# keith2018/TinyGPT

Hardware: AMD Instinct MI355X
Metric: decode tokens/sec (and % HBM roofline), Llama-3.2-1B bf16 batch=1, 1 GPU (higher is better)
Workload: dtype bf16; 1 GPU; Llama-3.2-1B bf16, batch 1 per GPU: 2048-token prefill then greedy decode (one step = one token, context 2054..3411); replicas=1, params=1235814400, graph=True

## Files before the change

### include/tgx.h

```cpp
#ifndef TGX_H
#define TGX_H

#include <stdint.h>

#ifdef __cplusplus
extern "C" {
#endif

#define TGX_ABI_VERSION 3

#if defined(__GNUC__)
#define TGX_API __attribute__((visibility("default")))
#else
#define TGX_API
#endif

typedef struct tgx_ctx tgx_ctx;

typedef enum tgx_status {
  TGX_OK = 0,
  TGX_ERR_INVALID = 1,
  TGX_ERR_UNSUPPORTED = 2,
  TGX_ERR_DEVICE = 3,
  TGX_ERR_STATE = 4,
// ... 132 lines not shown
#define TGX_KERNEL_LMHEAD 5
#define TGX_KERNEL_COUNT 6
TGX_API int tgx_profile_decode(tgx_ctx* ctx, int n_reps, int64_t* launches ,
                       double* total_ms );

TGX_API int tgx_read_probs(tgx_ctx* ctx, float* out);

TGX_API int tgx_set_logits(tgx_ctx* ctx, const float* logits, int batch);

TGX_API int tgx_set_option(tgx_ctx* ctx, const char* key, int value);

TGX_API int tgx_get_option(const tgx_ctx* ctx, const char* key, int* out_value);

TGX_API int64_t tgx_bytes_per_token(const tgx_ctx* ctx, int64_t T);

TGX_API int tgx_abi_version(void);

#ifdef __cplusplus
}
#endif
#endif
```

### tinygpt_amd/csrc/abi.hip

```cpp
#include <climits>
#include "ctx.h"
#include "kernels/kv_fork.h"
#include "kernels/kv_pack.h"
#include "row_snapshot.h"

static std::string g_create_err;

int set_err(tgx_ctx* c, int code, const char* fmt, ...) {
  char buf[512];
  va_list ap;
  va_start(ap, fmt);
  vsnprintf(buf, sizeof buf, fmt, ap);
  va_end(ap);
  if (c) c->err = buf; else g_create_err = buf;
  return code;
}

namespace {

inline uint16_t host_f32_to_bf16(float f) {
  uint32_t u;
  memcpy(&u, &f, 4);
  if ((u & 0x7fffffffu) > 0x7f800000u) return (uint16_t)((u >> 16) | 0x40);
  u += 0x7fffu + ((u >> 16) & 1u);
// ... 2093 lines not shown
  }
  return set_err(c, TGX_ERR_INVALID, "unknown option %s", key);
}

int64_t tgx_bytes_per_token(const tgx_ctx* c, int64_t T) {
  if (!c) return -1;
  const tgx_model_desc& d = c->d;
  const int64_t H = d.hidden, I = d.inter, V = d.vocab, L = d.layers, q = (int64_t)d.heads * d.head_dim, kv = (int64_t)d.kv_heads * d.head_dim;
  const int64_t b = (int64_t)c->esz;
  if (c->gpt2) {
    const int64_t per_layer = 3 * H * H + 3 * H + H * H + H + I * H + I + H * I + H + 4 * H;
    return b * (L * per_layer + 2 * H + H + V * H) + b * 2 * L * kv * T;
  }
  const int64_t per_layer = (q + 2 * kv) * H + (d.qkv_bias ? (q + 2 * kv) : 0) + H * q + 2 * I * H + H * I + 2 * H;
  int64_t saved = 0;
  auto packed_saving = [&](const PackedMat& m, int64_t rows, int64_t cols) { if (m.P) saved += b * rows * cols - rows * (m.row_bytes + 16); };
  for (const LayerW& w : c->L) { packed_saving(w.pgu, 2 * I, H); packed_saving(w.pdown, H, I); }
  packed_saving(c->plm, V, H);
  return b * (L * per_layer + H + V * H) + b * 2 * L * kv * T - saved;
}

}
```

### tinygpt_amd/csrc/ctx.h

```cpp
#pragma once
#include <hip/hip_runtime.h>

#include <algorithm>
#include <cmath>
#include <cstdarg>
#include <cstdio>
#include <cstdlib>
#include <cstring>
#include <string>
#include <vector>

#include "../../include/tgx.h"
#include "kernels/common.h"
#include "kv_pool.h"
#include "dev_mem.h"

using tgx::bf16_t;
typedef unsigned char ebyte;

namespace tgx { struct SampScratch; struct LpRecord; struct LpRow; }

constexpr int MAX_TICKET_EVENTS = 64;
constexpr int HOST_RING = 256;

struct PackedMat {
  unsigned char* P = nullptr;
  tgx::u32x4* rec = nullptr;
  long long row_bytes = 0;
  unsigned int base2 = 0;
  int ks = 0;
  int max_row_esc = 0;
  long long n_esc = 0;
};

struct LayerW {
  ebyte *in_norm = nullptr, *post_norm = nullptr;
  ebyte *wqkv = nullptr, *bqkv = nullptr, *wo = nullptr, *wgu = nullptr, *wdown = nullptr;
  PackedMat pgu, pdown;
  ebyte *q_norm = nullptr, *k_norm = nullptr;
  bool q_norm_ok = false, k_norm_ok = false;
  int merged_filled = 0;
  bool in_norm_ok = false, post_norm_ok = false, wo_ok = false, wdown_ok = false;
  ebyte *in_norm_b = nullptr, *post_norm_b = nullptr, *bo = nullptr, *bfc = nullptr, *bdown = nullptr;
  int gpt2_filled = 0;
// ... 260 lines not shown
template <typename T>
int dev_grow(tgx_ctx* c, T** p, size_t* bytes, size_t need) {
  if (need <= *bytes) return TGX_OK;
  HIP_OK(c, hipStreamSynchronize(c->stream));
  void* q = *p; const bool ok = c->mem.grow(&q, bytes, need); *p = static_cast<T*>(q);
  return ok ? TGX_OK : set_err(c, TGX_ERR_DEVICE, "dev_grow to %zu bytes failed: %s", need, hipGetErrorString(hipPeekAtLastError()));
}

namespace tgx { struct AttnArgs; struct FinalizeArgs; struct AttnPrefillArgs; struct RopeKvArgs; }

void drop_step_graphs(tgx_ctx* c);
int kv_ensure_blocks(tgx_ctx* c, int row, long long tokens);
bool is_greedy(const tgx_sampler_cfg* s);
bool row_records(const tgx_ctx* c, int row);
int gemv_grid(const tgx_ctx* c, int units, int ks, int bpc);
int pack_weights(tgx_ctx* c);
bool oproj_sliced_ok(const tgx_ctx* c, int R, long long kv_stride);
bool oproj_fused_capable(const tgx_ctx* c);
bool oproj_fused_ok(const tgx_ctx* c, int R, long long kv_stride);
int launch_layer_kernel(tgx_ctx* c, RowState* rv, int R, int l, int cls, float* resid, long long kv_stride);
void launch_layers(tgx_ctx* c, RowState* rv, int R, long long kv_stride);
void launch_layers(tgx_ctx* c, int row0, int R);
void launch_lm_head(tgx_ctx* c, int row0, int R);
void launch_lm_head_at(tgx_ctx* c, const float* x, float* logits, float* part_val, int* part_idx, int R);
tgx::FinalizeArgs make_finalize_args(tgx_ctx* c, int row, bool advance_pos, bool log_step);
void launch_finalize_greedy(tgx_ctx* c, int row0, int R, bool advance_pos, bool log_step);
void launch_finalize_rows(tgx_ctx* c, int row0, int M);
void launch_embed_chunk(tgx_ctx* c, const long long* ids, int R, int pos0);
void launch_add_pos(tgx_ctx* c, int* pos, int n);
void launch_argmax_partials(tgx_ctx* c, const float* logits, int V, float* part_val, int* part_idx);
// ... 47 lines not shown
```

### tinygpt_amd/csrc/decode.hip

```cpp
#include "ctx.h"
#include "kernels/attn_decode.h"
#include "kernels/gemv.h"
#include "kernels/gemv_packed.h"
#include "kernels/oproj_sliced.h"
#include "kernels/verify.h"

int gemv_grid(const tgx_ctx* c, int units, int ks, int bpc) {
  const int upb = 4 / ks;
  const int want = (units + upb - 1) / upb;
  const int cap = c->num_cus * bpc;
  return want < cap ? want : cap;
}

static int gemv_nx(int K, int ks) { return ((K / 8) + ks * 64 - 1) / (ks * 64); }

static int gemv_auto_ks(int K, int want) {
  int ks = want;
  while (ks < 4 && gemv_nx(K, ks) > 8) ks *= 2;
  return ks;
}

static tgx::GemvArgs gemv_row(const tgx_ctx* c, tgx::GemvArgs a, int r) {
  a.x += (size_t)r * a.x_stride;
  if (a.out) a.out += (size_t)r * a.out_stride;
// ... 20 lines not shown
  for (int r = 0; r < R; r++) hipLaunchKernelGGL((tgx::gemv_kernel<DT, PRO, EPI, NX, 1>), g, b, 0, c->stream, gemv_row(c, a, r));
}

template <int PRO, int EPI, int NX>
static void launch_gemv_packed_nx(tgx_ctx* c, const tgx::GemvPackedArgs& p, int grid) {
  const dim3 g(grid), b(256);
  if constexpr (EPI != tgx::EPI_LOGITS) {
    if (p.g.x_acc || p.g.res_acc) { hipLaunchKernelGGL((tgx::gemv_packed_kernel<PRO, EPI, NX, true>), g, b, p.g.x_acc ? (size_t)p.g.K * 4 : 0, c->stream, p); return; }
  }
  hipLaunchKernelGGL((tgx::gemv_packed_kernel<PRO, EPI, NX, false>), g, b, 0, c->stream, p);
}

template <int PRO, int EPI>
static void launch_gemv_packed(tgx_ctx* c, const tgx::GemvArgs& a, const PackedMat& pk, int grid, int nx) {
  tgx::GemvPackedArgs p{};
  p.g = a; p.P = pk.P; p.rec = pk.rec; p.row_bytes = pk.row_bytes; p.base2 = pk.base2;
  switch (nx) {
    case 1: launch_gemv_packed_nx<PRO, EPI, 1>(c, p, grid); break;
    case 2: launch_gemv_packed_nx<PRO, EPI, 2>(c, p, grid); break;
    case 3: launch_gemv_packed_nx<PRO, EPI, 3>(c, p, grid); break;
    case 4: launch_gemv_packed_nx<PRO, EPI, 4>(c, p, grid); break;
    case 5: launch_gemv_packed_nx<PRO, EPI, 5>(c, p, grid); break;
    case 6: launch_gemv_packed_nx<PRO, EPI, 6>(c, p, grid); break;
    case 7: launch_gemv_packed_nx<PRO, EPI, 7>(c, p, grid); break;
    default: launch_gemv_packed_nx<PRO, EPI, 8>(c, p, grid); break;
  }
}

static int pack_matrix(tgx_ctx* c, const ebyte* W, int N, int K, int cls, int* stat_dev, PackedMat* out) {
  const int ks = gemv_auto_ks(K, c->tune[cls].ks), nx = gemv_nx(K, ks);
  if (K % 8 || K > tgx::PACKED_K_MAX || nx > 8) return TGX_OK;
  PackedMat m;
  m.ks = ks; m.row_bytes = (long long)ks * ((nx + 3) / 4) * 3072;
  int rc;
  if ((rc = dev_alloc(c, &m.P, (size_t)N * (size_t)m.row_bytes)) || (rc = dev_alloc(c, &m.rec, (size_t)N))) { dev_free(c, &m.P); return rc; }
  HIP_OK(c, hipMemsetAsync(stat_dev, 0, 4 * sizeof(int), c->stream));
  const size_t n8 = (size_t)N * K / 8;
  hipLaunchKernelGGL(tgx::packed_maxexp_kernel, dim3((unsigned)std::min<size_t>((n8 + 255) / 256, 4096)), dim3(256), 0, c->stream, reinterpret_cast<const bf16_t*>(W), n8, stat_dev);
  tgx::PackRowsArgs a{};
  a.W = reinterpret_cast<const bf16_t*>(W); a.N = N; a.K = K; a.ks = ks; a.nx = nx; a.P = m.P; a.rec = m.rec; a.row_bytes = m.row_bytes; a.stat = stat_dev;
  hipLaunchKernelGGL(tgx::pack_rows_kernel, dim3(N), dim3(64), 0, c->stream, a);
  int stat[4] = {0, 0, 0, 0};
  HIP_OK(c, hipGetLastError());
  HIP_OK(c, hipMemcpyAsync(stat, stat_dev, sizeof(stat), hipMemcpyDeviceToHost, c->stream));
  HIP_OK(c, hipStreamSynchronize(c->stream));
  c->packed_max_row_esc = std::max(c->packed_max_row_esc, stat[3]);
  if (stat[1] > 0) {
    dev_free(c, &m.P); dev_free(c, &m.rec);
    c->packed_fallbacks++;
    return TGX_OK;
  }
  const unsigned int E0 = (unsigned int)std::max(stat[0] - 15, 0);
  m.base2 = (E0 << 7) | (E0 << 23); m.n_esc = stat[2]; m.max_row_esc = stat[3];
  *out = m;
  c->packed_matrices++;
  return TGX_OK;
}

int pack_weights(tgx_ctx* c) {
  const tgx_model_desc& d = c->d;
  if (!c->weights_packed || c->dt != tgx::DT_BF16 || c->gpt2) return TGX_OK;
  int* stat_dev = nullptr;
  int rc = dev_alloc(c, &stat_dev, 4);
  for (size_t l = 0; l < c->L.size() && !rc; l++) {
    LayerW& w = c->L[l];
    if (c->packed_classes & 1) rc = pack_matrix(c, w.wgu, 2 * d.inter, d.hidden, TGX_KERNEL_GATEUP, stat_dev, &w.pgu);
    if (!rc && (c->packed_classes & 2) && d.inter <= 16384) rc = pack_matrix(c, w.wdown, d.hidden, d.inter, TGX_KERNEL_DOWN, stat_dev, &w.pdown);
  }
  if (!rc && (c->packed_classes & 4)) rc = pack_matrix(c, d.tied ? c->embed : c->lm_head, d.vocab, d.hidden, TGX_KERNEL_LMHEAD, stat_dev, &c->plm);
  dev_free(c, &stat_dev);
// ... 254 lines not shown
```

### tinygpt_amd/csrc/kernels/gemv_packed.h

```cpp
#pragma once
#include "gemv.h"

namespace tgx {

constexpr int PACKED_ESC = 4;
constexpr int PACKED_K_MAX = 32768;

struct PackedQuad { u32x4 s01, s23, c; };

struct GemvPackedArgs {
  GemvArgs g;
  const unsigned char* P;
  const u32x4* rec;
  long long row_bytes;
  unsigned int base2;
};

__device__ __forceinline__ bool packed_has_escape(unsigned int C) { return ((C - 0x11111111u) & ~C & 0x88888888u) != 0; }

__device__ __forceinline__ Slice8<DT_BF16> packed_decode(unsigned int S0, unsigned int S1, unsigned int C, unsigned int base2, const u32x4 rec, int chunk) {
  Slice8<DT_BF16> o;
  o.v[0] = ((S0 & 0x007f007fu) | ((S0 << 8) & 0x80008000u)) + ((( C        & 0x000f000fu) << 7) + base2);
  o.v[1] = (((S0 >> 8) & 0x007f007fu) | (S0 & 0x80008000u)) + ((((C >> 4)  & 0x000f000fu) << 7) + base2);
  o.v[2] = ((S1 & 0x007f007fu) | ((S1 << 8) & 0x80008000u)) + ((((C >> 8)  & 0x000f000fu) << 7) + base2);
  o.v[3] = (((S1 >> 8) & 0x007f007fu) | (S1 & 0x80008000u)) + ((((C >> 12) & 0x000f000fu) << 7) + base2);
  if (packed_has_escape(C)) {
#pragma unroll
    for (int e = 0; e < PACKED_ESC; e++) {
      const unsigned int en = rec[e];
      const unsigned int t = (en >> 16) & 7u, sh = (t & 1u) << 4;
      const unsigned int dsel = (en >> 19) == (unsigned int)chunk ? (t >> 1) : 4u;
      const unsigned int m = 0xffffu << sh, val = (en & 0xffffu) << sh;
#pragma unroll
      for (int dd = 0; dd < 4; dd++) o.v[dd] = dsel == (unsigned int)dd ? ((o.v[dd] & ~m) | val) : o.v[dd];
    }
  }
  return o;
}

template <int PRO, int EPI, int NX, bool XACC = false>
__global__ __launch_bounds__(256, NX <= 4 ? 4 : 1) void gemv_packed_kernel(const GemvPackedArgs pa) {
  constexpr int DT = DT_BF16;
  constexpr int NQ = (NX + 3) / 4;
  typedef elem_t<DT> E;
  static_assert(PRO == PRO_PLAIN || PRO == PRO_RMSNORM, "packed forms: plain or RMSNorm prologue");
  static_assert(EPI == EPI_SILU_MUL || EPI == EPI_RESIDUAL || EPI == EPI_LOGITS, "packed forms: gate_up, down, lm_head");
  const GemvArgs& a = pa.g;
  const int n_wg = (int)gridDim.x;
  __shared__ float ps[4][2];
  __shared__ float sv[1][4];
  __shared__ int si[1][4];

  const int lane = threadIdx.x & 63, wv = threadIdx.x >> 6;
  const int KS = a.ks, UPB = 4 / KS;
  const int slot = wv / KS, kpart = wv - slot * KS;
  const int nchunk = a.K >> 3;
  const int per = ((nchunk + KS * 64 - 1) / (KS * 64)) * 64;
  const int c_begin = min(kpart * per, nchunk), c_end = min(c_begin + per, nchunk);
  const int stride = n_wg * UPB;

  int cidx[NX];
  bool cok[NX];
#pragma unroll
  for (int j = 0; j < NX; j++) {
    const int c = c_begin + lane + 64 * j;
    cok[j] = c < c_end;
    cidx[j] = cok[j] ? c : max(c_end - 1, 0);
  }

  const size_t lane_off = (size_t)kpart * NQ * 3072 + (size_t)lane * 16;
  PackedQuad wa[NQ], wb[NQ], na[NQ], nb[NQ];
  u32x4 ea, eb, nea = {}, neb = {};
  auto load_unit = [&](int ub, PackedQuad* ta, PackedQuad* tb, u32x4& ra_rec, u32x4& rb_rec) {
    const int u = min(ub + slot, a.units - 1);
    int ra, rb; bool v;
    unit_rows<EPI>(a, u, ra, rb, v);
    ra_rec = pa.rec[ra]; rb_rec = pa.rec[rb];
    const unsigned char* pra = pa.P + (size_t)ra * pa.row_bytes + lane_off;
    const unsigned char* prb = pa.P + (size_t)rb * pa.row_bytes + lane_off;
#pragma unroll
    for (int q = 0; q < NQ; q++) {
      const u32x4* qa = reinterpret_cast<const u32x4*>(pra + (size_t)q * 3072);
      const u32x4* qb = reinterpret_cast<const u32x4*>(prb + (size_t)q * 3072);
      ta[q].s01 = load_nt(qa); ta[q].s23 = load_nt(qa + 64); ta[q].c = load_nt(qa + 128);
      tb[q].s01 = load_nt(qb); tb[q].s23 = load_nt(qb + 64); tb[q].c = load_nt(qb + 128);
    }
  };
  auto rec_uniform = [](const u32x4 v) {
    return u32x4{(unsigned int)__builtin_amdgcn_readfirstlane((int)v[0]), (unsigned int)__builtin_amdgcn_readfirstlane((int)v[1]),
                 (unsigned int)__builtin_amdgcn_readfirstlane((int)v[2]), (unsigned int)__builtin_amdgcn_readfirstlane((int)v[3])};
  };

  float xr[NX][8];
  auto load_x = [&]() {
    const f32x4* xg = reinterpret_cast<const f32x4*>(a.x);
#pragma unroll
    for (int j = 0; j < NX; j++) {
      f32x4 v0 = xg[2 * cidx[j]], v1 = xg[2 * cidx[j] + 1];
      if (!cok[j]) { v0 = f32x4{0.f, 0.f, 0.f, 0.f}; v1 = v0; }
#pragma unroll
      for (int t = 0; t < 4; t++) { xr[j][t] = v0[t]; xr[j][4 + t] = v1[t]; }
    }
  };
  ulonglong2 xacc0[(XACC && PRO == PRO_RMSNORM) ? 4 : 1];
  if constexpr (XACC && PRO == PRO_RMSNORM) {
    const ulonglong2* ag = reinterpret_cast<const ulonglong2*>(a.x_acc + (size_t)min((int)threadIdx.x, nchunk - 1) * 8);
#pragma unroll
    for (int q = 0; q < 4; q++) xacc0[q] = ag[q];
    __builtin_amdgcn_sched_barrier(0);
  }
  int ub = blockIdx.x * UPB;
  if (ub < a.units) load_unit(ub, wa, wb, nea, neb);
  Slice8<DT> nw_x[(XACC && PRO == PRO_RMSNORM) ? NX : 1];
  if constexpr (XACC && PRO == PRO_RMSNORM) {
#pragma unroll
    for (int j = 0; j < NX; j++) nw_x[j] = load_slice<DT>(static_cast<const E*>(a.norm_w), cidx[j]);
    __builtin_amdgcn_sched_barrier(0);
  }

  if constexpr (XACC && PRO == PRO_RMSNORM) {
    extern __shared__ __attribute__((aligned(16))) float xs[];
    for (int cs = threadIdx.x; cs < nchunk; cs += 256) {
      ulonglong2 t[4];
      if (cs == (int)threadIdx.x) {
#pragma unroll
        for (int q = 0; q < 4; q++) t[q] = xacc0[q];
      } else {
// ... 46 lines not shown
      slice_unpack<DT>(nw[j], w);
#pragma unroll
      for (int t = 0; t < 8; t++) xr[j][t] = w[t] * (xr[j][t] * inv);
    }
  }

  if constexpr (PRO != PRO_PLAIN) {
    if (a.act16) {
#pragma unroll
      for (int j = 0; j < NX; j++)
#pragma unroll
        for (int t = 0; t < 8; t++) xr[j][t] = elem_to_f32<DT>(f32_to_elem<DT>(xr[j][t]));
    }
  }

  float best_val = -INFINITY;
  int best_idx = 0x7fffffff;
  ea = rec_uniform(nea); eb = rec_uniform(neb);

  for (; ub < a.units; ub += stride) {
    const bool has_next = ub + stride < a.units;
    if (has_next) load_unit(ub + stride, na, nb, nea, neb);

    const int u = ub + slot;
    const bool writer = u < a.units && kpart == 0 && lane == 0;
    int ra = 0, rb = 0; bool rb_valid = false;
    float e0 = 0.f, e1 = 0.f;
    if (writer) {
      unit_rows<EPI>(a, u, ra, rb, rb_valid);
      if (EPI == EPI_RESIDUAL) {
        if constexpr (XACC) { e0 = fix_to_f32(a.res_acc[ra]); e1 = fix_to_f32(a.res_acc[rb]); }
        else { e0 = a.out[ra]; e1 = a.out[rb]; }
      }
    }

    float acc_a0 = 0.f, acc_b0 = 0.f, acc_a1 = 0.f, acc_b1 = 0.f;
#pragma unroll
    for (int j = 0; j < NX; j++) {
      const f32x4 xa = f32x4{xr[j][0], xr[j][1], xr[j][2], xr[j][3]};
      const f32x4 xb = f32x4{xr[j][4], xr[j][5], xr[j][6], xr[j][7]};
      const int q = j >> 2, jj = j & 3;
      const u32x4 sa4 = (jj & 2) ? wa[q].s23 : wa[q].s01, sb4 = (jj & 2) ? wb[q].s23 : wb[q].s01;
      const int chunk = c_begin + lane + 64 * j;
      const Slice8<DT> da = packed_decode(sa4[(jj & 1) * 2], sa4[(jj & 1) * 2 + 1], wa[q].c[jj], pa.base2, ea, chunk);
      const Slice8<DT> db = packed_decode(sb4[(jj & 1) * 2], sb4[(jj & 1) * 2 + 1], wb[q].c[jj], pa.base2, eb, chunk);
      if (j & 1) { acc_a1 = dot8<DT>(acc_a1, da, xa, xb); acc_b1 = dot8<DT>(acc_b1, db, xa, xb); }
      else       { acc_a0 = dot8<DT>(acc_a0, da, xa, xb); acc_b0 = dot8<DT>(acc_b0, db, xa, xb); }
    }
    float sa = wave_sum(acc_a0 + acc_a1);
    float sb = wave_sum(acc_b0 + acc_b1);

    if (KS > 1) {
      __syncthreads();
      if (lane == 0) { ps[wv][0] = sa; ps[wv][1] = sb; }
      __syncthreads();
      if (kpart == 0) {
        sa = ps[slot * KS][0]; sb = ps[slot * KS][1];
        for (int k = 1; k < KS; k++) { sa += ps[slot * KS + k][0]; sb += ps[slot * KS + k][1]; }
      }
    }

    if (writer) {
      float va = sa, vb = sb;
      if (EPI == EPI_LOGITS) {
        a.logits[ra] = va;
// ... 2 lines not shown
          a.logits[rb] = vb;
          if (vb > best_val) { best_val = vb; best_idx = rb; }
        }
      } else {
        if (a.bias) { const E* bias = static_cast<const E*>(a.bias); va += elem_to_f32<DT>(bias[ra]); vb += elem_to_f32<DT>(bias[rb]); }
        if (EPI == EPI_RESIDUAL) {
          a.out[ra] = e0 + va;
          if (rb_valid) a.out[rb] = e1 + vb;
          if constexpr (XACC) { a.res_acc[ra] = 0; if (rb_valid) a.res_acc[rb] = 0; }
        } else if (EPI == EPI_SILU_MUL) {
          a.out[u] = round_storage_if<DT>((va / (1.0f + expf(-va))) * vb, a.act16);
        }
      }
    }

#pragma unroll
    for (int q = 0; q < NQ; q++) { wa[q] = na[q]; wb[q] = nb[q]; }
    ea = rec_uniform(nea); eb = rec_uniform(neb);
  }

  if (EPI == EPI_LOGITS) {
    if (lane == 0) { sv[0][wv] = best_val; si[0][wv] = best_idx; }
    __syncthreads();
    if (threadIdx.x == 0) {
      float bv = sv[0][0]; int bi = si[0][0];
      for (int w = 1; w < 4; w++)
        if (sv[0][w] > bv || (sv[0][w] == bv && si[0][w] < bi)) { bv = sv[0][w]; bi = si[0][w]; }
      a.part_val[blockIdx.x] = bv;
      a.part_idx[blockIdx.x] = bi;
    }
  }
}

// ... 3 lines not shown
    const u32x4 v = reinterpret_cast<const u32x4*>(W)[i];
#pragma unroll
    for (int t = 0; t < 4; t++) {
      const int e0 = (v[t] >> 7) & 0xff, e1 = (v[t] >> 23) & 0xff;
      if (e0 < 255) m = max(m, e0);
      if (e1 < 255) m = max(m, e1);
    }
  }
#pragma unroll
  for (int o = 32; o > 0; o >>= 1) m = max(m, __shfl_xor(m, o, 64));
  if ((threadIdx.x & 63) == 0) atomicMax(stat, m);
}

struct PackRowsArgs {
  const bf16_t* W;
  int N, K, ks, nx;
  unsigned char* P;
  u32x4* rec;
  long long row_bytes;
  int* stat;
};

__global__ __launch_bounds__(64) void pack_rows_kernel(const PackRowsArgs a) {
  __shared__ unsigned int ent[PACKED_ESC];
  const int row = blockIdx.x, lane = threadIdx.x;
  const int E0 = max(a.stat[0] - 15, 0);
  const bf16_t* w = a.W + (size_t)row * a.K;
  if (lane < PACKED_ESC) ent[lane] = 0xffffffffu;
  __syncthreads();
  int cnt = 0;
  for (int k0 = 0; k0 < a.K; k0 += 64) {
    const int k = k0 + lane;
    unsigned int bits = 0; bool esc = false;
    if (k < a.K) { bits = w[k]; const int code = (int)((bits >> 7) & 0xff) - E0; esc = code < 1 || code > 15; }
    const unsigned long long bal = __ballot(esc);
    const int p = cnt + __popcll(bal & ((1ull << lane) - 1ull));
    if (esc && p < PACKED_ESC) ent[p] = ((unsigned int)k << 16) | bits;
    cnt += __popcll(bal);
  }
  __syncthreads();
  if (lane == 0) {
    a.rec[row] = u32x4{ent[0], ent[1], ent[2], ent[3]};
    if (cnt > PACKED_ESC) atomicAdd(a.stat + 1, 1);
    if (cnt) { atomicAdd(a.stat + 2, cnt); atomicMax(a.stat + 3, cnt); }
  }
  const int nchunk = a.K >> 3, nq = (a.nx + 3) / 4;
  const int per = ((nchunk + a.ks * 64 - 1) / (a.ks * 64)) * 64;
  for (int p = 0; p < a.ks; p++) {
    const int c_begin = min(p * per, nchunk), c_end = min(c_begin + per, nchunk);
    for (int q = 0; q < nq; q++) {
      unsigned int S[8], C[4];
#pragma unroll
      for (int jj = 0; jj < 4; jj++) {
        const int j = 4 * q + jj, c = c_begin + lane + 64 * j;
        S[2 * jj] = 0; S[2 * jj + 1] = 0; C[jj] = 0x11111111u;
        if (j < a.nx && c < c_end) {
          const u32x4 v = reinterpret_cast<const u32x4*>(w)[c];
          unsigned int b[8], cd[8];
#pragma unroll
          for (int t = 0; t < 8; t++) {
            const unsigned int bits = (v[t >> 1] >> (16 * (t & 1))) & 0xffffu;
            const int code = (int)((bits >> 7) & 0xff) - E0;
            b[t] = ((bits >> 8) & 0x80u) | (bits & 0x7fu);
            cd[t] = (code < 1 || code > 15) ? 0u : (unsigned int)code;
          }
          S[2 * jj] = b[0] | (b[2] << 8) | (b[1] << 16) | (b[3] << 24);
          S[2 * jj + 1] = b[4] | (b[6] << 8) | (b[5] << 16) | (b[7] << 24);
          unsigned int cc = 0;
#pragma unroll
          for (int t = 0; t < 4; t++) cc |= (cd[2 * t] << (4 * t)) | (cd[2 * t + 1] << (4 * t + 16));
          C[jj] = cc;
        }
      }
      u32x4* dst = reinterpret_cast<u32x4*>(a.P + (size_t)row * a.row_bytes + ((size_t)p * nq + q) * 3072) + lane;
      dst[0] = u32x4{S[0], S[1], S[2], S[3]};
      dst[64] = u32x4{S[4], S[5], S[6], S[7]};
      dst[128] = u32x4{C[0], C[1], C[2], C[3]};
    }
  }
}

}
```

### tinygpt_amd/ffi.py

```python
from __future__ import annotations

import ctypes
import os
from ctypes import POINTER, c_char_p, c_double, c_float, c_int, c_int32, c_int64, c_uint64, c_void_p

import numpy as np

from .desc import CDesc, ModelDesc, DTYPE_BF16, DTYPE_F32, DTYPE_F16
from . import synth

HERE = os.path.dirname(os.path.abspath(__file__))
PRODUCT_LIB = os.path.join(HERE, "lib", "libtgx_mi355x.so")

STATUS_NAMES = {0: "TGX_OK", 1: "TGX_ERR_INVALID", 2: "TGX_ERR_UNSUPPORTED", 3: "TGX_ERR_DEVICE", 4: "TGX_ERR_STATE",
                5: "TGX_ERR_NOMEM", 6: "TGX_ERR_NAME", 7: "TGX_ERR_SHAPE", 8: "TGX_ERR_CONTEXT"}

MAX_LOGPROBS, LOGPROB_RING = 20, 256
KERNEL_CLASSES = ["qkv", "attn", "oproj", "gateup", "down", "lmhead"]


class SamplerCfg(ctypes.Structure):
    _fields_ = [("temperature", c_float), ("top_k", c_int64), ("top_p", c_float), ("min_p", c_float)]

    def __init__(self, temperature=0.0, top_k=0, top_p=1.0, min_p=0.0):
# ... 58 lines not shown
    "set_row_penalties": (c_int, [c_void_p, c_int, POINTER(PenaltyCfg)]),
    "set_row_logit_bias": (c_int, [c_void_p, c_int, c_int, POINTER(c_int32), POINTER(c_float)]),
    "set_row_history": (c_int, [c_void_p, c_int, POINTER(c_int64), c_int, POINTER(c_int64), c_int]),
    "context_size": (c_int64, [c_void_p]),
    "num_layers": (c_int32, [c_void_p]),
    "last_error": (c_char_p, [c_void_p]),
    "synchronize": (c_int, [c_void_p]),
    "read_kv": (c_int, [c_void_p, c_int, c_int, POINTER(c_float), POINTER(c_float)]),
    "write_kv": (c_int, [c_void_p, c_int, c_int, POINTER(c_float), POINTER(c_float), c_int64]),
    "profile_decode": (c_int, [c_void_p, c_int, POINTER(c_int64), POINTER(c_double)]),
    "set_option": (c_int, [c_void_p, c_char_p, c_int]),
    "get_option": (c_int, [c_void_p, c_char_p, POINTER(c_int)]),
    "read_probs": (c_int, [c_void_p, POINTER(c_float)]),
    "set_logits": (c_int, [c_void_p, POINTER(c_float), c_int]),
    "bytes_per_token": (c_int64, [c_void_p, c_int64]),
    "abi_version": (c_int, []),
}


class Backend:

    def __init__(self, path: str, prefix: str = "tgx_", required=None, extra=None):
        if not os.path.exists(path):
            raise FileNotFoundError(
                f"{path} not found — build it first (python -c 'import __graft_entry__ as g; g.build()'). "
                "tinygpt_amd has no CPU fallback.")
        self.path = path
        self.prefix = prefix
        self.lib = ctypes.CDLL(path, mode=ctypes.RTLD_LOCAL)
        table = dict(ABI)
# ... 304 lines not shown
        self._check(self.be.set_logits(self._ctx, l.ctypes.data_as(POINTER(c_float)), l.shape[0]))
        self.batch = l.shape[0]
        return self

    def set_option(self, key: str, value: int):
        self._check(self.be.set_option(self._ctx, key.encode(), int(value)))
        return self

    def get_option(self, key: str) -> int:
        out = c_int(0)
        self._check(self.be.get_option(self._ctx, key.encode(), ctypes.byref(out)))
        return out.value

    def bytes_per_token(self, T: int) -> int:
        return self.be.bytes_per_token(self._ctx, T)
```

Baseline: 1554 tokens/s.

## Repack compressed weights into fp8-style paired-row units with hardware fp8 decode

Changes the 12-bit packed bf16 weight format. Each weight's high byte now holds sign, a 4-bit exponent code and 3 mantissa bits, so the hardware fp8-to-f32 scaled convert can decode it, and the remaining 4 mantissa bits go in a separate nibble plane. Two rows are interleaved per unit and accumulated with packed f32 FMAs, and the gemv loop double-buffers by alternating two unit buffers. Escape records grow from 4 per row to a K-dependent cap of up to 32, repaired via readlane, so more matrices can stay packed. The aim is to cut ALU work in the bandwidth-bound decode GEMVs, at the cost of a more complex escape-repair path. A debug readback entry point is also added.

Result: slower. 1539 tokens/s (-1.0%).

```diff
diff --git a/include/tgx.h b/include/tgx.h
--- a/include/tgx.h
+++ b/include/tgx.h
@@ -170,6 +170,8 @@
 
 TGX_API int64_t tgx_bytes_per_token(const tgx_ctx* ctx, int64_t T);
 
+TGX_API int tgx_debug_packed_readback(tgx_ctx* ctx, const char* name, uint16_t* out_bits, int64_t count);
+
 TGX_API int tgx_abi_version(void);
 
 #ifdef __cplusplus
diff --git a/tinygpt_amd/csrc/abi.hip b/tinygpt_amd/csrc/abi.hip
--- a/tinygpt_amd/csrc/abi.hip
+++ b/tinygpt_amd/csrc/abi.hip
@@ -2131,10 +2131,25 @@
   }
   const int64_t per_layer = (q + 2 * kv) * H + (d.qkv_bias ? (q + 2 * kv) : 0) + H * q + 2 * I * H + H * I + 2 * H;
   int64_t saved = 0;
-  auto packed_saving = [&](const PackedMat& m, int64_t rows, int64_t cols) { if (m.P) saved += b * rows * cols - rows * (m.row_bytes + 16); };
+  auto packed_saving = [&](const PackedMat& m, int64_t rows, int64_t cols) { if (m.P) saved += b * rows * cols - (m.units * m.unit_bytes + rows * m.rec_cap * 4); };
   for (const LayerW& w : c->L) { packed_saving(w.pgu, 2 * I, H); packed_saving(w.pdown, H, I); }
   packed_saving(c->plm, V, H);
   return b * (L * per_layer + H + V * H) + b * 2 * L * kv * T - saved;
 }
 
-}
+int tgx_debug_packed_readback(tgx_ctx* c, const char* name, uint16_t* out_bits, int64_t count) {
+  if (!c) return TGX_ERR_INVALID;
+  if (!name || !out_bits) return set_err(c, TGX_ERR_INVALID, "tgx_debug_packed_readback: null argument");
+  if (!c->finalized) return set_err(c, TGX_ERR_STATE, "tgx_debug_packed_readback after tgx_finalize (the packed copies are made there)");
+  const PackedMat* m = nullptr;
+  int l = -1, n = 0;
+  if (!strcmp(name, "lm_head")) m = &c->plm;
+  else if (sscanf(name, "layers.%d.gate_up%n", &l, &n) == 1 && n && !name[n]) { if (l >= 0 && l < (int)c->L.size()) m = &c->L[l].pgu; }
+  else if (sscanf(name, "layers.%d.down%n", &l, &n) == 1 && n && !name[n]) { if (l >= 0 && l < (int)c->L.size()) m = &c->L[l].pdown; }
+  if (!m) return set_err(c, TGX_ERR_INVALID, "tgx_debug_packed_readback: no matrix %s (lm_head, layers.<l>.gate_up, layers.<l>.down)", name);
+  if (!m->P) return set_err(c, TGX_ERR_STATE, "matrix %s is not stored packed", name);
+  if (count != (int64_t)m->N * m->K) return set_err(c, TGX_ERR_INVALID, "matrix %s holds %d x %d weights, the buffer %lld", name, m->N, m->K, (long long)count);
+  return packed_readback(c, *m, out_bits);
+}
+
+}
diff --git a/tinygpt_amd/csrc/ctx.h b/tinygpt_amd/csrc/ctx.h
--- a/tinygpt_amd/csrc/ctx.h
+++ b/tinygpt_amd/csrc/ctx.h
@@ -25,9 +25,12 @@
 
 struct PackedMat {
   unsigned char* P = nullptr;
-  tgx::u32x4* rec = nullptr;
-  long long row_bytes = 0;
-  unsigned int base2 = 0;
+  unsigned int* rec = nullptr;
+  long long unit_bytes = 0;
+  float scale = 0.f;
+  int N = 0, K = 0, nx = 0, units = 0;
+  int split = 0;
+  int rec_cap = 0;
   int ks = 0;
   int max_row_esc = 0;
   long long n_esc = 0;
@@ -318,6 +321,7 @@
 bool is_greedy(const tgx_sampler_cfg* s);
 bool row_records(const tgx_ctx* c, int row);
 int gemv_grid(const tgx_ctx* c, int units, int ks, int bpc);
+int packed_readback(tgx_ctx* c, const PackedMat& m, unsigned short* out);
 int pack_weights(tgx_ctx* c);
 bool oproj_sliced_ok(const tgx_ctx* c, int R, long long kv_stride);
 bool oproj_fused_capable(const tgx_ctx* c);
diff --git a/tinygpt_amd/csrc/decode.hip b/tinygpt_amd/csrc/decode.hip
--- a/tinygpt_amd/csrc/decode.hip
+++ b/tinygpt_amd/csrc/decode.hip
@@ -58,7 +58,7 @@
 template <int PRO, int EPI>
 static void launch_gemv_packed(tgx_ctx* c, const tgx::GemvArgs& a, const PackedMat& pk, int grid, int nx) {
   tgx::GemvPackedArgs p{};
-  p.g = a; p.P = pk.P; p.rec = pk.rec; p.row_bytes = pk.row_bytes; p.base2 = pk.base2;
+  p.g = a; p.P = pk.P; p.rec = pk.rec; p.unit_bytes = pk.unit_bytes; p.scale = pk.scale; p.rec_cap = pk.rec_cap;
   switch (nx) {
     case 1: launch_gemv_packed_nx<PRO, EPI, 1>(c, p, grid); break;
     case 2: launch_gemv_packed_nx<PRO, EPI, 2>(c, p, grid); break;
@@ -71,19 +71,26 @@
   }
 }
 
+static tgx::PackRowsArgs pack_rows_args(const PackedMat& m, const ebyte* W, int* stat_dev) {
+  tgx::PackRowsArgs a{};
+  a.W = reinterpret_cast<const bf16_t*>(W); a.N = m.N; a.K = m.K; a.ks = m.ks; a.nx = m.nx; a.split = m.split; a.units = m.units; a.rec_cap = m.rec_cap;
+  a.P = m.P; a.rec = m.rec; a.unit_bytes = m.unit_bytes; a.stat = stat_dev;
+  return a;
+}
+
 static int pack_matrix(tgx_ctx* c, const ebyte* W, int N, int K, int cls, int* stat_dev, PackedMat* out) {
   const int ks = gemv_auto_ks(K, c->tune[cls].ks), nx = gemv_nx(K, ks);
   if (K % 8 || K > tgx::PACKED_K_MAX || nx > 8) return TGX_OK;
   PackedMat m;
-  m.ks = ks; m.row_bytes = (long long)ks * ((nx + 3) / 4) * 3072;
+  m.N = N; m.K = K; m.nx = nx; m.ks = ks; m.split = cls == TGX_KERNEL_GATEUP; m.units = m.split ? N / 2 : (N + 1) / 2;
+  m.unit_bytes = (long long)ks * ((nx + 1) / 2) * 3072; m.rec_cap = tgx::packed_rec_cap(K);
   int rc;
-  if ((rc = dev_alloc(c, &m.P, (size_t)N * (size_t)m.row_bytes)) || (rc = dev_alloc(c, &m.rec, (size_t)N))) { dev_free(c, &m.P); return rc; }
+  if ((rc = dev_alloc(c, &m.P, (size_t)m.units * (size_t)m.unit_bytes)) || (rc = dev_alloc(c, &m.rec, (size_t)N * m.rec_cap))) { dev_free(c, &m.P); return rc; }
   HIP_OK(c, hipMemsetAsync(stat_dev, 0, 4 * sizeof(int), c->stream));
   const size_t n8 = (size_t)N * K / 8;
   hipLaunchKernelGGL(tgx::packed_maxexp_kernel, dim3((unsigned)std::min<size_t>((n8 + 255) / 256, 4096)), dim3(256), 0, c->stream, reinterpret_cast<const bf16_t*>(W), n8, stat_dev);
-  tgx::PackRowsArgs a{};
-  a.W = reinterpret_cast<const bf16_t*>(W); a.N = N; a.K = K; a.ks = ks; a.nx = nx; a.P = m.P; a.rec = m.rec; a.row_bytes = m.row_bytes; a.stat = stat_dev;
-  hipLaunchKernelGGL(tgx::pack_rows_kernel, dim3(N), dim3(64), 0, c->stream, a);
+  const tgx::PackRowsArgs a = pack_rows_args(m, W, stat_dev);
+  hipLaunchKernelGGL(tgx::pack_rows_kernel, dim3(m.units), dim3(64), 0, c->stream, a);
   int stat[4] = {0, 0, 0, 0};
   HIP_OK(c, hipGetLastError());
   HIP_OK(c, hipMemcpyAsync(stat, stat_dev, sizeof(stat), hipMemcpyDeviceToHost, c->stream));
@@ -94,10 +101,22 @@
     c->packed_fallbacks++;
     return TGX_OK;
   }
-  const unsigned int E0 = (unsigned int)std::max(stat[0] - 15, 0);
-  m.base2 = (E0 << 7) | (E0 << 23); m.n_esc = stat[2]; m.max_row_esc = stat[3];
+  m.scale = ldexpf(1.0f, std::max(stat[0] - 15, 0) - 120); m.n_esc = stat[2]; m.max_row_esc = stat[3];
   *out = m;
   c->packed_matrices++;
+  return TGX_OK;
+}
+
+int packed_readback(tgx_ctx* c, const PackedMat& m, unsigned short* out) {
+  bf16_t* dev = nullptr;
+  int rc = dev_alloc(c, &dev, (size_t)m.N * m.K);
+  if (rc) return rc;
+  hipLaunchKernelGGL(tgx::packed_readback_kernel, dim3(m.units), dim3(64), 0, c->stream, pack_rows_args(m, nullptr, nullptr), m.scale, dev);
+  hipError_t e = hipGetLastError();
+  if (e == hipSuccess) e = hipMemcpyAsync(out, dev, (size_t)m.N * m.K * sizeof(bf16_t), hipMemcpyDeviceToHost, c->stream);
+  if (e == hipSuccess) e = hipStreamSynchronize(c->stream);
+  dev_free(c, &dev);
+  HIP_OK(c, e);
   return TGX_OK;
 }
 
diff --git a/tinygpt_amd/csrc/kernels/gemv_packed.h b/tinygpt_amd/csrc/kernels/gemv_packed.h
--- a/tinygpt_amd/csrc/kernels/gemv_packed.h
+++ b/tinygpt_amd/csrc/kernels/gemv_packed.h
@@ -4,44 +4,88 @@
 namespace tgx {
 
 constexpr int PACKED_ESC = 4;
+constexpr int PACKED_ESC_COLS = 2048;
+constexpr int PACKED_REC_MAX = 32;
 constexpr int PACKED_K_MAX = 32768;
-
-struct PackedQuad { u32x4 s01, s23, c; };
+constexpr unsigned int PACKED_EMPTY = 0xffffffffu;
+
+__host__ __device__ inline int packed_rec_cap(int K) {
+  const int c = PACKED_ESC * ((K + PACKED_ESC_COLS - 1) / PACKED_ESC_COLS);
+  return c < PACKED_REC_MAX ? c : PACKED_REC_MAX;
+}
+__host__ __device__ inline void packed_unit_rows(int u, int N, int split, int& ra, int& rb) {
+  if (split) { ra = u; rb = u + (N >> 1); }
+  else { ra = 2 * u; rb = ra + 1 < N ? ra + 1 : ra; }
+}
+
+typedef float f32x2 __attribute__((ext_vector_type(2)));
+
+template <int NX> struct PackedUnit { u32x4 lo[(NX + 1) / 2], hi[NX]; };
 
 struct GemvPackedArgs {
   GemvArgs g;
   const unsigned char* P;
-  const u32x4* rec;
-  long long row_bytes;
-  unsigned int base2;
+  const unsigned int* rec;
+  long long unit_bytes;
+  float scale;
+  int rec_cap;
 };
 
-__device__ __forceinline__ bool packed_has_escape(unsigned int C) { return ((C - 0x11111111u) & ~C & 0x88888888u) != 0; }
-
-__device__ __forceinline__ Slice8<DT_BF16> packed_decode(unsigned int S0, unsigned int S1, unsigned int C, unsigned int base2, const u32x4 rec, int chunk) {
-  Slice8<DT_BF16> o;
-  o.v[0] = ((S0 & 0x007f007fu) | ((S0 << 8) & 0x80008000u)) + ((( C        & 0x000f000fu) << 7) + base2);
-  o.v[1] = (((S0 >> 8) & 0x007f007fu) | (S0 & 0x80008000u)) + ((((C >> 4)  & 0x000f000fu) << 7) + base2);
-  o.v[2] = ((S1 & 0x007f007fu) | ((S1 << 8) & 0x80008000u)) + ((((C >> 8)  & 0x000f000fu) << 7) + base2);
-  o.v[3] = (((S1 >> 8) & 0x007f007fu) | (S1 & 0x80008000u)) + ((((C >> 12) & 0x000f000fu) << 7) + base2);
-  if (packed_has_escape(C)) {
-#pragma unroll
-    for (int e = 0; e < PACKED_ESC; e++) {
-      const unsigned int en = rec[e];
-      const unsigned int t = (en >> 16) & 7u, sh = (t & 1u) << 4;
-      const unsigned int dsel = (en >> 19) == (unsigned int)chunk ? (t >> 1) : 4u;
-      const unsigned int m = 0xffffu << sh, val = (en & 0xffffu) << sh;
-#pragma unroll
-      for (int dd = 0; dd < 4; dd++) o.v[dd] = dsel == (unsigned int)dd ? ((o.v[dd] & ~m) | val) : o.v[dd];
-    }
-  }
-  return o;
+__device__ __forceinline__ f32x2 packed_fma_lo(f32x2 w, f32x2 x, f32x2 acc) {
+  asm("v_pk_fma_f32 %0, %1, %2, %0 op_sel_hi:[1,0,1]" : "+v"(acc) : "v"(w), "v"(x));
+  return acc;
+}
+__device__ __forceinline__ f32x2 packed_fma_hi(f32x2 w, f32x2 x, f32x2 acc) {
+  asm("v_pk_fma_f32 %0, %1, %2, %0 op_sel:[0,1,0]" : "+v"(acc) : "v"(w), "v"(x));
+  return acc;
+}
+
+__device__ __forceinline__ void packed_decode8(const u32x4 H, unsigned int lo_a, unsigned int lo_b, float scale, f32x2 w[8]) {
+#pragma unroll
+  for (int i = 0; i < 4; i++) {
+    w[2 * i] = __builtin_amdgcn_cvt_scalef32_pk_f32_fp8(H[i], scale, false);
+    w[2 * i + 1] = __builtin_amdgcn_cvt_scalef32_pk_f32_fp8(H[i], scale, true);
+  }
+#pragma unroll
+  for (int t = 0; t < 8; t++) {
+    const int pos = 4 * ((t + 4) & 7);
+    const unsigned int na = pos >= 16 ? lo_a >> (pos - 16) : lo_a << (16 - pos);
+    const unsigned int nb = pos >= 16 ? lo_b >> (pos - 16) : lo_b << (16 - pos);
+    w[t].x = __uint_as_float((na & 0x000f0000u) | __float_as_uint(w[t].x));
+    w[t].y = __uint_as_float((nb & 0x000f0000u) | __float_as_uint(w[t].y));
+  }
+}
+
+__device__ __forceinline__ void packed_repair8(f32x2 w[8], unsigned int recv, int rec_cap, int c0, int lane) {
+#pragma unroll
+  for (int h = 0; h < 2; h++) {
+    for (int e = 0; e < rec_cap; e++) {
+      const unsigned int en = (unsigned int)__builtin_amdgcn_readlane((int)recv, h * 32 + e);
+      if (en == PACKED_EMPTY) break;
+      const int rel = (int)(en >> 19) - c0;
+      if ((unsigned int)rel < 64u) {
+        const unsigned int tsel = (en >> 16) & 7u;
+        const float val = __uint_as_float(en << 16);
+#pragma unroll
+        for (int t = 0; t < 8; t++) {
+          const bool m = lane == rel && tsel == (unsigned int)t;
+          if (h == 0) w[t].x = m ? val : w[t].x; else w[t].y = m ? val : w[t].y;
+        }
+      }
+    }
+  }
+}
+__device__ __forceinline__ bool packed_any_escape(unsigned int recv) {
+  return (((unsigned int)__builtin_amdgcn_readlane((int)recv, 0) & (unsigned int)__builtin_amdgcn_readlane((int)recv, 32)) >> 31) == 0u;
+}
+__device__ __forceinline__ unsigned int packed_load_rec(const unsigned int* rec, int rec_cap, int ra, int rb, int lane) {
+  return rec[(size_t)(lane < 32 ? ra : rb) * rec_cap + min(lane & 31, rec_cap - 1)];
 }
 
 template <int PRO, int EPI, int NX, bool XACC = false>
 __global__ __launch_bounds__(256, NX <= 4 ? 4 : 1) void gemv_packed_kernel(const GemvPackedArgs pa) {
   constexpr int DT = DT_BF16;
-  constexpr int NQ = (NX + 3) / 4;
+  constexpr int NP = (NX + 1) / 2;
   typedef elem_t<DT> E;
   static_assert(PRO == PRO_PLAIN || PRO == PRO_RMSNORM, "packed forms: plain or RMSNorm prologue");
   static_assert(EPI == EPI_SILU_MUL || EPI == EPI_RESIDUAL || EPI == EPI_LOGITS, "packed forms: gate_up, down, lm_head");
@@ -58,6 +102,7 @@
   const int per = ((nchunk + KS * 64 - 1) / (KS * 64)) * 64;
   const int c_begin = min(kpart * per, nchunk), c_end = min(c_begin + per, nchunk);
   const int stride = n_wg * UPB;
+  const int c_begin_u = __builtin_amdgcn_readfirstlane(c_begin);
 
   int cidx[NX];
   bool cok[NX];
@@ -68,27 +113,21 @@
     cidx[j] = cok[j] ? c : max(c_end - 1, 0);
   }
 
-  const size_t lane_off = (size_t)kpart * NQ * 3072 + (size_t)lane * 16;
-  PackedQuad wa[NQ], wb[NQ], na[NQ], nb[NQ];
-  u32x4 ea, eb, nea = {}, neb = {};
-  auto load_unit = [&](int ub, PackedQuad* ta, PackedQuad* tb, u32x4& ra_rec, u32x4& rb_rec) {
+  const size_t lane_off = (size_t)kpart * NP * 3072 + (size_t)lane * 16;
+  PackedUnit<NX> wA, wB;
+  unsigned int recA = PACKED_EMPTY, recB = PACKED_EMPTY;
+  auto load_unit = [&](int ub, bool valid, PackedUnit<NX>& t, unsigned int& trec) {
     const int u = min(ub + slot, a.units - 1);
     int ra, rb; bool v;
     unit_rows<EPI>(a, u, ra, rb, v);
-    ra_rec = pa.rec[ra]; rb_rec = pa.rec[rb];
-    const unsigned char* pra = pa.P + (size_t)ra * pa.row_bytes + lane_off;
-    const unsigned char* prb = pa.P + (size_t)rb * pa.row_bytes + lane_off;
-#pragma unroll
-    for (int q = 0; q < NQ; q++) {
-      const u32x4* qa = reinterpret_cast<const u32x4*>(pra + (size_t)q * 3072);
-      const u32x4* qb = reinterpret_cast<const u32x4*>(prb + (size_t)q * 3072);
-      ta[q].s01 = load_nt(qa); ta[q].s23 = load_nt(qa + 64); ta[q].c = load_nt(qa + 128);
-      tb[q].s01 = load_nt(qb); tb[q].s23 = load_nt(qb + 64); tb[q].c = load_nt(qb + 128);
-    }
-  };
-  auto rec_uniform = [](const u32x4 v) {
-    return u32x4{(unsigned int)__builtin_amdgcn_readfirstlane((int)v[0]), (unsigned int)__builtin_amdgcn_readfirstlane((int)v[1]),
-                 (unsigned int)__builtin_amdgcn_readfirstlane((int)v[2]), (unsigned int)__builtin_amdgcn_readfirstlane((int)v[3])};
+    trec = packed_load_rec(pa.rec, pa.rec_cap, ra, rb, lane);
+    const u32x4* p = reinterpret_cast<const u32x4*>(valid ? pa.P + (size_t)u * pa.unit_bytes + lane_off : pa.P);
+#pragma unroll
+    for (int q = 0; q < NP; q++) {
+      t.lo[q] = load_nt(p + q * 192);
+      t.hi[2 * q] = load_nt(p + q * 192 + 64);
+      if (2 * q + 1 < NX) t.hi[2 * q + 1] = load_nt(p + q * 192 + 128);
+    }
   };
 
   float xr[NX][8];
@@ -110,7 +149,7 @@
     __builtin_amdgcn_sched_barrier(0);
   }
   int ub = blockIdx.x * UPB;
-  if (ub < a.units) load_unit(ub, wa, wb, nea, neb);
+  load_unit(ub, ub < a.units, wA, recA);
   Slice8<DT> nw_x[(XACC && PRO == PRO_RMSNORM) ? NX : 1];
   if constexpr (XACC && PRO == PRO_RMSNORM) {
 #pragma unroll
@@ -187,13 +226,17 @@
     }
   }
 
+  f32x2 xp[NX][4];
+#pragma unroll
+  for (int j = 0; j < NX; j++)
+#pragma unroll
+    for (int i = 0; i < 4; i++) xp[j][i] = f32x2{xr[j][2 * i], xr[j][2 * i + 1]};
+
   float best_val = -INFINITY;
   int best_idx = 0x7fffffff;
-  ea = rec_uniform(nea); eb = rec_uniform(neb);
-
-  for (; ub < a.units; ub += stride) {
-    const bool has_next = ub + stride < a.units;
-    if (has_next) load_unit(ub + stride, na, nb, nea, neb);
+
+  auto unit_step = [&](const PackedUnit<NX>& cur, const unsigned int crec, PackedUnit<NX>& nxt, unsigned int& nrec) {
+    load_unit(ub + stride, ub + stride < a.units, nxt, nrec);
 
     const int u = ub + slot;
     const bool writer = u < a.units && kpart == 0 && lane == 0;
@@ -207,21 +250,23 @@
       }
     }
 
-    float acc_a0 = 0.f, acc_b0 = 0.f, acc_a1 = 0.f, acc_b1 = 0.f;
+    const bool fix = packed_any_escape(crec);
+    f32x2 acc0 = {0.f, 0.f}, acc1 = {0.f, 0.f};
 #pragma unroll
     for (int j = 0; j < NX; j++) {
-      const f32x4 xa = f32x4{xr[j][0], xr[j][1], xr[j][2], xr[j][3]};
-      const f32x4 xb = f32x4{xr[j][4], xr[j][5], xr[j][6], xr[j][7]};
-      const int q = j >> 2, jj = j & 3;
-      const u32x4 sa4 = (jj & 2) ? wa[q].s23 : wa[q].s01, sb4 = (jj & 2) ? wb[q].s23 : wb[q].s01;
-      const int chunk = c_begin + lane + 64 * j;
-      const Slice8<DT> da = packed_decode(sa4[(jj & 1) * 2], sa4[(jj & 1) * 2 + 1], wa[q].c[jj], pa.base2, ea, chunk);
-      const Slice8<DT> db = packed_decode(sb4[(jj & 1) * 2], sb4[(jj & 1) * 2 + 1], wb[q].c[jj], pa.base2, eb, chunk);
-      if (j & 1) { acc_a1 = dot8<DT>(acc_a1, da, xa, xb); acc_b1 = dot8<DT>(acc_b1, db, xa, xb); }
-      else       { acc_a0 = dot8<DT>(acc_a0, da, xa, xb); acc_b0 = dot8<DT>(acc_b0, db, xa, xb); }
-    }
-    float sa = wave_sum(acc_a0 + acc_a1);
-    float sb = wave_sum(acc_b0 + acc_b1);
+      f32x2 w[8];
+      packed_decode8(cur.hi[j], cur.lo[j >> 1][(j & 1) * 2], cur.lo[j >> 1][(j & 1) * 2 + 1], pa.scale, w);
+      if (fix) packed_repair8(w, crec, pa.rec_cap, c_begin_u + 64 * j, lane);
+      f32x2 acc = (j & 1) ? acc1 : acc0;
+#pragma unroll
+      for (int i = 0; i < 4; i++) {
+        acc = packed_fma_lo(w[2 * i], xp[j][i], acc);
+        acc = packed_fma_hi(w[2 * i + 1], xp[j][i], acc);
+      }
+      if (j & 1) acc1 = acc; else acc0 = acc;
+    }
+    float sa = wave_sum(acc0.x + acc1.x);
+    float sb = wave_sum(acc0.y + acc1.y);
 
     if (KS > 1) {
       __syncthreads();
@@ -254,9 +299,13 @@
       }
     }
 
-#pragma unroll
-    for (int q = 0; q < NQ; q++) { wa[q] = na[q]; wb[q] = nb[q]; }
-    ea = rec_uniform(nea); eb = rec_uniform(neb);
+  };
+  while (ub < a.units) {
+    unit_step(wA, recA, wB, recB);
+    ub += stride;
+    if (ub >= a.units) break;
+    unit_step(wB, recB, wA, recA);
+    ub += stride;
   }
 
   if (EPI == EPI_LOGITS) {
@@ -290,70 +339,110 @@
 
 struct PackRowsArgs {
   const bf16_t* W;
-  int N, K, ks, nx;
+  int N, K, ks, nx, split, units, rec_cap;
   unsigned char* P;
-  u32x4* rec;
-  long long row_bytes;
+  unsigned int* rec;
+  long long unit_bytes;
   int* stat;
 };
 
+__device__ __forceinline__ bool packed_is_escape(unsigned int bits, int E0) {
+  const int code = (int)((bits >> 7) & 0xff) - E0;
+  return code < 1 || code > 15 || (code == 15 && (bits & 0x70u) == 0x70u);
+}
+
 __global__ __launch_bounds__(64) void pack_rows_kernel(const PackRowsArgs a) {
-  __shared__ unsigned int ent[PACKED_ESC];
-  const int row = blockIdx.x, lane = threadIdx.x;
+  __shared__ unsigned int ent[PACKED_REC_MAX];
+  const int u = blockIdx.x, lane = threadIdx.x;
   const int E0 = max(a.stat[0] - 15, 0);
-  const bf16_t* w = a.W + (size_t)row * a.K;
-  if (lane < PACKED_ESC) ent[lane] = 0xffffffffu;
-  __syncthreads();
-  int cnt = 0;
-  for (int k0 = 0; k0 < a.K; k0 += 64) {
-    const int k = k0 + lane;
-    unsigned int bits = 0; bool esc = false;
-    if (k < a.K) { bits = w[k]; const int code = (int)((bits >> 7) & 0xff) - E0; esc = code < 1 || code > 15; }
-    const unsigned long long bal = __ballot(esc);
-    const int p = cnt + __popcll(bal & ((1ull << lane) - 1ull));
-    if (esc && p < PACKED_ESC) ent[p] = ((unsigned int)k << 16) | bits;
-    cnt += __popcll(bal);
-  }
-  __syncthreads();
-  if (lane == 0) {
-    a.rec[row] = u32x4{ent[0], ent[1], ent[2], ent[3]};
-    if (cnt > PACKED_ESC) atomicAdd(a.stat + 1, 1);
-    if (cnt) { atomicAdd(a.stat + 2, cnt); atomicMax(a.stat + 3, cnt); }
-  }
-  const int nchunk = a.K >> 3, nq = (a.nx + 3) / 4;
+  int ra, rb;
+  packed_unit_rows(u, a.N, a.split, ra, rb);
+  for (int h = 0; h < (rb != ra ? 2 : 1); h++) {
+    const int row = h ? rb : ra;
+    const bf16_t* w = a.W + (size_t)row * a.K;
+    __syncthreads();
+    if (lane < PACKED_REC_MAX) ent[lane] = PACKED_EMPTY;
+    __syncthreads();
+    int cnt = 0;
+    for (int k0 = 0; k0 < a.K; k0 += 64) {
+      const int k = k0 + lane;
+      unsigned int bits = 0; bool esc = false;
+      if (k < a.K) { bits = w[k]; esc = packed_is_escape(bits, E0); }
+      const unsigned long long bal = __ballot(esc);
+      const int p = cnt + __popcll(bal & ((1ull << lane) - 1ull));
+      if (esc && p < a.rec_cap) ent[p] = ((unsigned int)k << 16) | bits;
+      cnt += __popcll(bal);
+    }
+    __syncthreads();
+    if (lane < a.rec_cap) a.rec[(size_t)row * a.rec_cap + lane] = ent[lane];
+    if (lane == 0) {
+      if (cnt > a.rec_cap) atomicAdd(a.stat + 1, 1);
+      if (cnt) { atomicAdd(a.stat + 2, cnt); atomicMax(a.stat + 3, cnt); }
+    }
+  }
+  const bf16_t* wra = a.W + (size_t)ra * a.K;
+  const bf16_t* wrb = a.W + (size_t)rb * a.K;
+  const int nchunk = a.K >> 3, np = (a.nx + 1) / 2;
   const int per = ((nchunk + a.ks * 64 - 1) / (a.ks * 64)) * 64;
   for (int p = 0; p < a.ks; p++) {
     const int c_begin = min(p * per, nchunk), c_end = min(c_begin + per, nchunk);
-    for (int q = 0; q < nq; q++) {
-      unsigned int S[8], C[4];
-#pragma unroll
-      for (int jj = 0; jj < 4; jj++) {
-        const int j = 4 * q + jj, c = c_begin + lane + 64 * j;
-        S[2 * jj] = 0; S[2 * jj + 1] = 0; C[jj] = 0x11111111u;
+    for (int q = 0; q < np; q++) {
+      unsigned int H[8] = {0, 0, 0, 0, 0, 0, 0, 0}, L[4] = {0, 0, 0, 0};
+#pragma unroll
+      for (int jj = 0; jj < 2; jj++) {
+        const int j = 2 * q + jj, c = c_begin + lane + 64 * j;
         if (j < a.nx && c < c_end) {
-          const u32x4 v = reinterpret_cast<const u32x4*>(w)[c];
-          unsigned int b[8], cd[8];
+          const u32x4 va = reinterpret_cast<const u32x4*>(wra)[c], vb = reinterpret_cast<const u32x4*>(wrb)[c];
 #pragma unroll
           for (int t = 0; t < 8; t++) {
-            const unsigned int bits = (v[t >> 1] >> (16 * (t & 1))) & 0xffffu;
-            const int code = (int)((bits >> 7) & 0xff) - E0;
-            b[t] = ((bits >> 8) & 0x80u) | (bits & 0x7fu);
-            cd[t] = (code < 1 || code > 15) ? 0u : (unsigned int)code;
+#pragma unroll
+            for (int h = 0; h < 2; h++) {
+              const unsigned int bits = ((h ? vb : va)[t >> 1] >> (16 * (t & 1))) & 0xffffu;
+              const bool esc = packed_is_escape(bits, E0);
+              const unsigned int code = (bits >> 7 & 0xffu) - (unsigned int)E0;
+              const unsigned int hb = esc ? (bits >> 8) & 0x80u : ((bits >> 8) & 0x80u) | (code << 3) | ((bits >> 4) & 7u);
+              const unsigned int nib = esc ? 0u : bits & 15u;
+              H[4 * jj + (t >> 1)] |= hb << (16 * (t & 1) + 8 * h);
+              L[2 * jj + h] |= nib << (4 * ((t + 4) & 7));
+            }
           }
-          S[2 * jj] = b[0] | (b[2] << 8) | (b[1] << 16) | (b[3] << 24);
-          S[2 * jj + 1] = b[4] | (b[6] << 8) | (b[5] << 16) | (b[7] << 24);
-          unsigned int cc = 0;
-#pragma unroll
-          for (int t = 0; t < 4; t++) cc |= (cd[2 * t] << (4 * t)) | (cd[2 * t + 1] << (4 * t + 16));
-          C[jj] = cc;
         }
       }
-      u32x4* dst = reinterpret_cast<u32x4*>(a.P + (size_t)row * a.row_bytes + ((size_t)p * nq + q) * 3072) + lane;
-      dst[0] = u32x4{S[0], S[1], S[2], S[3]};
-      dst[64] = u32x4{S[4], S[5], S[6], S[7]};
-      dst[128] = u32x4{C[0], C[1], C[2], C[3]};
-    }
-  }
-}
-
-}
+      u32x4* dst = reinterpret_cast<u32x4*>(a.P + (size_t)u * a.unit_bytes + ((size_t)p * np + q) * 3072) + lane;
+      dst[0] = u32x4{L[0], L[1], L[2], L[3]};
+      dst[64] = u32x4{H[0], H[1], H[2], H[3]};
+      dst[128] = u32x4{H[4], H[5], H[6], H[7]};
+    }
+  }
+}
+
+__global__ __launch_bounds__(64) void packed_readback_kernel(const PackRowsArgs a, float scale, bf16_t* out) {
+  const int u = blockIdx.x, lane = threadIdx.x;
+  int ra, rb;
+  packed_unit_rows(u, a.N, a.split, ra, rb);
+  const unsigned int recv = packed_load_rec(a.rec, a.rec_cap, ra, rb, lane);
+  const bool fix = packed_any_escape(recv);
+  const int nchunk = a.K >> 3, np = (a.nx + 1) / 2;
+  const int per = ((nchunk + a.ks * 64 - 1) / (a.ks * 64)) * 64;
+  for (int p = 0; p < a.ks; p++) {
+    const int c_begin = min(p * per, nchunk), c_end = min(c_begin + per, nchunk);
+    for (int j = 0; j < a.nx; j++) {
+      const u32x4* src = reinterpret_cast<const u32x4*>(a.P + (size_t)u * a.unit_bytes + ((size_t)p * np + (j >> 1)) * 3072) + lane;
+      const u32x4 lo = src[0], hi = src[64 * (1 + (j & 1))];
+      f32x2 w[8];
+      packed_decode8(hi, (j & 1) ? lo[2] : lo[0], (j & 1) ? lo[3] : lo[1], scale, w);
+      if (fix) packed_repair8(w, recv, a.rec_cap, c_begin + 64 * j, lane);
+      const int c = c_begin + lane + 64 * j;
+      if (c < c_end) {
+#pragma unroll
+        for (int t = 0; t < 8; t++) {
+          const unsigned int fa = __float_as_uint(w[t].x), fb = __float_as_uint(w[t].y);
+          out[(size_t)ra * a.K + 8 * c + t] = (bf16_t)((fa & 0xffffu) ? ~(fa >> 16) : fa >> 16);
+          out[(size_t)rb * a.K + 8 * c + t] = (bf16_t)((fb & 0xffffu) ? ~(fb >> 16) : fb >> 16);
+        }
+      }
+    }
+  }
+}
+
+}
diff --git a/tinygpt_amd/ffi.py b/tinygpt_amd/ffi.py
--- a/tinygpt_amd/ffi.py
+++ b/tinygpt_amd/ffi.py
@@ -96,6 +96,7 @@
     "read_probs": (c_int, [c_void_p, POINTER(c_float)]),
     "set_logits": (c_int, [c_void_p, POINTER(c_float), c_int]),
     "bytes_per_token": (c_int64, [c_void_p, c_int64]),
+    "debug_packed_readback": (c_int, [c_void_p, c_char_p, POINTER(ctypes.c_uint16), c_int64]),
     "abi_version": (c_int, []),
 }
 
@@ -430,3 +431,8 @@
 
     def bytes_per_token(self, T: int) -> int:
         return self.be.bytes_per_token(self._ctx, T)
+
+    def packed_readback(self, name: str, rows: int, cols: int) -> np.ndarray:
+        out = np.empty((rows, cols), dtype=np.uint16)
+        self._check(self.be.debug_packed_readback(self._ctx, name.encode(), out.ctypes.data_as(POINTER(ctypes.c_uint16)), out.size))
+        return out
```
